# dtarb/TauDEM

Measured on AMD Instinct MI355X. Metric: Mcells/s (PitRemove->D8FlowDir->AreaD8 pipeline), higher is better.
Workload: dtype f32

## Files before the change

### taudem_amd/csrc/pitremove.hip

```cpp
#include "context.hpp"
#include "device_common.hpp"
#include "strips.hpp"
#include "tile_relax.hpp"

namespace {

constexpr int SEED_ROWS = 16;
constexpr int SEED_CF = 8;
template <int MODE>
__global__ __launch_bounds__(256) void pit_seed_kernel(const float* __restrict__ Z, const int16_t* __restrict__ mask,
                                                       float* __restrict__ W, int nx, int ny, int y_own0, int y_own1, float nodata, int step,
                                                       float* __restrict__ Zc, float* __restrict__ Wc, int nxc, int nyc, int nbx, int xmap) {
    const int bx = tdxk::xcd_block_x(nbx, xmap);
    if (bx < 0) return;
    const int x = bx * 64 + (threadIdx.x & 63);
    const int ybase = y_own0 + blockIdx.y * (4 * SEED_ROWS) + (threadIdx.x >> 6) * SEED_ROWS;
    const bool colok = x < nx;
    const int xc = colok ? x : nx - 1, xm = xc > 0 ? xc - 1 : xc, xp = xc < nx - 1 ? xc + 1 : xc;
    const int lane = int(threadIdx.x & 63);
    const bool edge_lane = lane == 0 || lane == 63;
    const int xe = lane == 0 ? xm : xp;
    float zm[SEED_ROWS + 2], zedge[SEED_ROWS + 2];
#pragma unroll
    for (int j = 0; j < SEED_ROWS + 2; j++) {
// ... 20 lines not shown
        const int l = tilek::lane_left(c, 0), r = tilek::lane_right(c, 0);
        nod[j] = in ? (unsigned(lane == 0 ? e : l) | (unsigned(c) << 1) | (unsigned(lane == 63 ? e : r) << 2)) : 7u;
    }
    float bmax[SEED_ROWS / SEED_CF];
    bool bany[SEED_ROWS / SEED_CF], bseed[SEED_ROWS / SEED_CF];
#pragma unroll
    for (int q = 0; q < SEED_ROWS / SEED_CF; q++) { bmax[q] = -FLT_MAX; bany[q] = false; bseed[q] = false; }
#pragma unroll
    for (int r = 0; r < SEED_ROWS; r++) {
        const int y = ybase + r;
        const float zc = zm[r + 1];
        const unsigned nn = nod[r], nc = nod[r + 1], ns = nod[r + 2];
        const bool c1 = (nc & 2u) != 0u;
        if (colok && y < y_own1) {
            const size_t idx = size_t(y) * size_t(nx) + size_t(x);
            float w;
            if (c1) w = TDX_FEL_NODATA;
            else if (mask && mask[idx] == 1) w = zc;
            else if (x == 0 || y == 0 || x == nx - 1 || y == ny - 1) w = zc;
            else {
                const bool con = (step == 2) ? (((nc & 5u) | (nn & 2u) | (ns & 2u)) != 0u) : ((nn | nc | ns) != 0u);
                w = con ? zc : FLT_MAX;
            }
            if (MODE == 0) W[idx] = w;
            if (MODE == 1 && !c1) {
                bany[r / SEED_CF] = true;
                bmax[r / SEED_CF] = fmaxf(bmax[r / SEED_CF], zc);
                if (w != FLT_MAX) bseed[r / SEED_CF] = true;
            }
            if (MODE == 2) {
                if (w == FLT_MAX) w = wc[r / SEED_CF];
                W[idx] = w;
            }
        }
    }
    if (MODE == 1) {
#pragma unroll
        for (int q = 0; q < SEED_ROWS / SEED_CF; q++) {
            float m = bmax[q];
            int fl = (bany[q] ? 1 : 0) | (bseed[q] ? 2 : 0);
#pragma unroll
            for (int off = 1; off < SEED_CF; off <<= 1) {
                m = fmaxf(m, __shfl_xor(m, off, 64));
                fl |= __shfl_xor(fl, off, 64);
            }
            const int yc = (ybase - y_own0) / SEED_CF + q, xcb = x / SEED_CF;
            if ((threadIdx.x & (SEED_CF - 1)) == 0 && xcb < nxc && yc < nyc) {
                const size_t c = size_t(yc) * size_t(nxc) + size_t(xcb);
                Zc[c] = (fl & 1) ? m : TDX_FEL_NODATA;
                Wc[c] = (fl & 1) ? ((fl & 2) ? m : FLT_MAX) : TDX_FEL_NODATA;
            }
        }
    }
}

constexpr int CF = 8;
static_assert(CF == SEED_CF, "pit_seed_kernel reduces to the first coarse level");
__global__ __launch_bounds__(256) void pit_coarsen_kernel(const float* __restrict__ Z, const float* __restrict__ W0, int nx, int ny, int nxc, int nyc,
                                                          float* __restrict__ Zc, float* __restrict__ Wc) {
// ... 89 lines not shown

template <int NBR>
struct PitOp {
    using T = float;
    static constexpr int kUniform = NBR;
    static constexpr int kWaves = 5;
    const float* Z;
    float* W;
    static __device__ __forceinline__ float inf() { return FLT_MAX; }
    using Raw = float;
    using CellRaw = float;
    __device__ __forceinline__ float load_raw(size_t idx) const { return W[idx]; }
    static __device__ __forceinline__ float decode(float v) { return v; }
    __device__ __forceinline__ void store(size_t idx, float v) const { W[idx] = v; }
    __device__ __forceinline__ float cell_raw(size_t idx) const { return Z[idx]; }
    static __device__ __forceinline__ void cell_decode(float z, float& cst, unsigned& mask) { cst = z; mask = (NBR == 4) ? 0x55u : 0xFFu; }
    static __device__ __forceinline__ float cell_floor(float z, float w) { return (w > z) ? z : w; }
    static __device__ __forceinline__ float apply(float z, float w, float m) { return tilek::med3_raw(z, w, m); }
    static __device__ __forceinline__ bool settled(float z, float w) { return !(w > z); }
    static __device__ __forceinline__ float act_never() { return -FLT_MAX; }
    static __device__ __forceinline__ float act_threshold(float z, float w) { return (w > z) ? w : act_never(); }
};

}

static int pit_finish_level(tdx_context* ctx, const Strip& ls, float* Zc, float* Wc, int nxc, int nyc, int64_t cells_all, tilek::Sched sc, int depth,
                            int64_t* rounds, int64_t* launches, int64_t* own_rounds = nullptr);

static inline Strip pit_level_strip(const Strip& st, int nxc, int nyc) {
    Strip ls;
    ls.nx = nxc; ls.comm = st.comm;
    if (st.multi()) { ls.ny_arr = nyc + 2; ls.y0 = 1; ls.y1 = nyc + 1; ls.up = st.up; ls.down = st.down; }
    else { ls.ny_arr = nyc; ls.y0 = 0; ls.y1 = nyc; }
    return ls;
}

template <int NBR>
static int pit_relax_level(tdx_context* ctx, const Strip& ls, const float* Z, float* W, tilek::Sched sc, int64_t* rounds, int64_t* launches, int64_t* outer,
                           bool all_tiles = true) {
    const tilek::TileGeom g = tilek::make_geom(ls.nx, ls.ny_arr, ls.y0, ls.y1);
    for (;;) {
        int rc = tile_relax_run(ctx, PitOp<NBR>{Z, W}, g, sc, rounds, launches, all_tiles);
        all_tiles = false;
        if (rc != TDX_OK) return rc;
        if (outer) (*outer)++;
        if (!ls.multi()) break;
        int64_t changed = 0;
        rc = strip_exchange<float>(ctx, ls, W, TDX_FEL_NODATA, sc.flags, g.tiles_x, &changed, true);
        if (rc != TDX_OK) return rc;
        if (changed == 0) break;
    }
    return TDX_OK;
}

static int pit_coarse_start(tdx_context* ctx, const Strip& st, const float* Z, float* W, int nx, int nyo, int64_t cells_all, tilek::Sched sc, int depth,
                            int64_t* rounds, int64_t* launches) {
    if (depth >= 3 || cells_all < (int64_t(1) << 18) || nyo < 1) return TDX_OK;
    hipStream_t s = ctx->stream;
    const int nxc = (nx + CF - 1) / CF, nyc = (nyo + CF - 1) / CF;
    const Strip ls = pit_level_strip(st, nxc, nyc);
    const size_t nc = size_t(nxc) * size_t(ls.ny_arr), off = size_t(ls.y0) * size_t(nxc);
    float* Zc = static_cast<float*>(ctx->scratch(TDX_S_D + 2 * depth, nc * 4));
    float* Wc = static_cast<float*>(ctx->scratch(TDX_S_E + 2 * depth, nc * 4));
    if (!Zc || !Wc) return TDX_ERR_NOMEM;
    const dim3 gc((nxc + 63) / 64, (nyc + 3) / 4);
// ... 24 lines not shown
    TDX_HIP_CHECK(ctx, hipSetDevice(ctx->device));
    hipStream_t s = ctx->stream;
    const tilek::TileGeom geom = tilek::make_geom(st.nx, st.ny_arr, st.y0, st.y1);
    const int ntiles = geom.tiles_x * geom.tiles_y;
    uint32_t* flags = static_cast<uint32_t*>(ctx->scratch(TDX_S_A, size_t(ntiles) * 4));
    uint32_t* list = static_cast<uint32_t*>(ctx->scratch(TDX_S_B, size_t(ntiles) * 4 * tilek::SCHED_LIST_WORDS));
    unsigned long long* counts = static_cast<unsigned long long*>(ctx->scratch(TDX_S_C, size_t(tilek::COUNT_RING) * 16));
    if (!flags || !list || !counts) return TDX_ERR_NOMEM;
    const tilek::Sched sched{flags, list, counts};

    ctx->begin_call(stats);
    strip_mark(ctx, st, "pitremove");
    int rc = strip_exchange<float>(ctx, st, d_dem, dem_nodata);
    if (rc != TDX_OK) return rc;
    int64_t rounds = 0, launches = 0, outer = 0;
    const int sbx = (st.nx + 63) / 64, sxmap = 0;
    const dim3 sgrid(unsigned(sbx), (st.y1 - st.y0 + 4 * SEED_ROWS - 1) / (4 * SEED_ROWS));
    const bool no_coarse = getenv("TDX_PIT_NO_COARSE") != nullptr;
    const int nyo = st.y1 - st.y0;
    int64_t cells_all = int64_t(st.nx) * int64_t(nyo);
    rc = strip_allreduce(ctx, st, &cells_all, 1, TDX_OP_SUM);
    if (rc != TDX_OK) return rc;
    const bool used_coarse = !fourway && !no_coarse && cells_all >= (int64_t(1) << 18);
    int64_t level1_rounds = 0;
    if (used_coarse) {
        const int nxc = (st.nx + CF - 1) / CF, nyc = (nyo + CF - 1) / CF;
        const Strip ls = pit_level_strip(st, nxc, nyc);
        const size_t nc = size_t(nxc) * size_t(ls.ny_arr), off = size_t(ls.y0) * size_t(nxc);
        float* Zc = static_cast<float*>(ctx->scratch(TDX_S_D, nc * 4));
        float* Wc = static_cast<float*>(ctx->scratch(TDX_S_E, nc * 4));
        if (!Zc || !Wc) return TDX_ERR_NOMEM;
        {
            TdxSpan sp(ctx, TDX_K_STENCIL);
            hipLaunchKernelGGL(pit_seed_kernel<1>, sgrid, dim3(256), 0, s, d_dem, d_mask, d_fel, st.nx, st.ny_arr, st.y0, st.y1, dem_nodata, 1, Zc + off, Wc + off, nxc, nyc, sbx, sxmap);
            if (stats) stats->launches[TDX_K_STENCIL]++;
        }
        {
            TdxSpan sp(ctx, TDX_K_RELAX);
            ctx->phase = "coarse levels";
            rc = pit_finish_level(ctx, ls, Zc, Wc, nxc, nyc, cells_all / (CF * CF), sched, 0, &rounds, &launches, &level1_rounds);
            if (rc != TDX_OK) return rc;
        }
        {
            TdxSpan sp(ctx, TDX_K_STENCIL);
            hipLaunchKernelGGL(pit_seed_kernel<2>, sgrid, dim3(256), 0, s, d_dem, d_mask, d_fel, st.nx, st.ny_arr, st.y0, st.y1, dem_nodata, 1, Zc + off, Wc + off, nxc, nyc, sbx, sxmap);
            if (stats) stats->launches[TDX_K_STENCIL]++;
        }
    } else {
        TdxSpan sp(ctx, TDX_K_STENCIL);
        hipLaunchKernelGGL(pit_seed_kernel<0>, sgrid, dim3(256), 0, s, d_dem, d_mask, d_fel, st.nx, st.ny_arr, st.y0, st.y1, dem_nodata, fourway ? 2 : 1,
                           static_cast<float*>(nullptr), static_cast<float*>(nullptr), 0, 0, sbx, sxmap);
        if (stats) stats->launches[TDX_K_STENCIL]++;
    }
    ctx->phase = "fine level";
    rc = strip_exchange<float>(ctx, st, d_fel, TDX_FEL_NODATA);
    if (rc != TDX_OK) return rc;
    {
        TdxSpan sp(ctx, TDX_K_RELAX);
        bool all_tiles = true;
        const int vc_env = getenv("TDX_PIT_VCYCLE_AFTER") ? std::max(0, atoi(getenv("TDX_PIT_VCYCLE_AFTER"))) : 8;
        if (used_coarse && vc_env > 0) {
            bool left = false;
            rc = tile_relax_run_bounded(ctx, PitOp<8>{d_dem, d_fel}, geom, sched, vc_env, &left, &rounds, &launches, true);
            if (rc != TDX_OK) return rc;
            all_tiles = false;
            const int vc_min = getenv("TDX_PIT_VCYCLE_MIN") ? atoi(getenv("TDX_PIT_VCYCLE_MIN")) : 16;
            if (st.multi() || (left && level1_rounds >= vc_min)) {
                const int nxc = (st.nx + CF - 1) / CF, nyc = (nyo + CF - 1) / CF;
                const Strip ls = pit_level_strip(st, nxc, nyc);
                const size_t off = size_t(ls.y0) * size_t(nxc);
                float* Zc = static_cast<float*>(ctx->scratch(TDX_S_D, size_t(nxc) * size_t(ls.ny_arr) * 4));
                float* Wc = static_cast<float*>(ctx->scratch(TDX_S_E, size_t(nxc) * size_t(ls.ny_arr) * 4));
                const tilek::TileGeom gc = tilek::make_geom(ls.nx, ls.ny_arr, ls.y0, ls.y1);
                const size_t ntc = size_t(gc.tiles_x) * size_t(gc.tiles_y);
                uint32_t* cflags = static_cast<uint32_t*>(ctx->scratch(TDX_S_L, ntc * 4 * (1 + tilek::SCHED_LIST_WORDS)));
                unsigned long long* ccounts = static_cast<unsigned long long*>(ctx->scratch(TDX_S_M, size_t(tilek::COUNT_RING) * 16));
                float* Ur = static_cast<float*>(ctx->scratch(TDX_S_N, size_t(nxc) * size_t(nyc) * 4));
                if (!Zc || !Wc || !cflags || !ccounts || !Ur) return TDX_ERR_NOMEM;
                ctx->phase = "coarse correction";
                TDX_HIP_CHECK(ctx, hipMemsetAsync(cflags, 0, ntc * 4, s));
                hipLaunchKernelGGL(pit_restrict_kernel, dim3((nxc + 63) / 64, (nyc + 3) / 4), dim3(256), 0, s, d_fel + size_t(st.y0) * size_t(st.nx), st.nx, nyo, nxc, nyc, Wc + off, Ur,
                                   ls.y0, ls.ny_arr, gc.tiles_x, cflags);
                {
                    int64_t changed = 0;
                    rc = strip_exchange<float>(ctx, ls, Wc, TDX_FEL_NODATA, cflags, gc.tiles_x, &changed);
                    if (rc != TDX_OK) return rc;
                }
                rc = pit_relax_level<8>(ctx, ls, Zc, Wc, tilek::Sched{cflags, cflags + ntc, ccounts}, &rounds, &launches, nullptr, false);
                if (rc != TDX_OK) return rc;
                hipLaunchKernelGGL(pit_prolong_min_kernel, dim3((st.nx + 63) / 64, (nyc + 3) / 4), dim3(256), 0, s, d_fel + size_t(st.y0) * size_t(st.nx), st.nx, nyo, Wc + off, Ur, nxc, nyc,
                                   st.y0, st.ny_arr, geom.tiles_x, flags);
                ctx->phase = "fine level";
                if (st.multi()) {
                    int64_t changed = 0;
                    rc = strip_exchange<float>(ctx, st, d_fel, TDX_FEL_NODATA, flags, geom.tiles_x, &changed);
                    if (rc != TDX_OK) return rc;
                }
            }
        }
        rc = fourway ? pit_relax_level<4>(ctx, st, d_dem, d_fel, sched, &rounds, &launches, &outer, all_tiles) : pit_relax_level<8>(ctx, st, d_dem, d_fel, sched, &rounds, &launches, &outer, all_tiles);
        if (rc != TDX_OK) return rc;
        if (stats) stats->launches[TDX_K_RELAX] += launches;
    }
    TDX_HIP_CHECK(ctx, hipGetLastError());
    if (stats) { stats->rounds = rounds; stats->cells_evaluated = outer; }
    ctx->end_call();
    return TDX_OK;
}

static int pitremove_check(tdx_context* ctx, const void* dem, const void* fel, int64_t nx, int64_t ny, int64_t halo, const char* who) {
    if (!ctx || !dem || !fel || nx <= 0 || ny <= 0) return tdx_fail(ctx, TDX_ERR_ARG, who);
    return too_big(nx, ny + halo) ? tdx_fail(ctx, TDX_ERR_ARG, "raster larger than 2^32 cells per device strip") : TDX_OK;
}

extern "C" int tdx_pitremove_dev(tdx_context* ctx, const float* d_dem, int64_t nx, int64_t ny, float dem_nodata,
                                 const int16_t* d_mask, int fourway, float* d_fel, tdx_stats* stats) {
    if (int rc = pitremove_check(ctx, d_dem, d_fel, nx, ny, 0, "tdx_pitremove_dev: bad argument")) return rc;
    return pitremove_impl(ctx, strip_single(int(nx), int(ny)), const_cast<float*>(d_dem), d_mask, fourway, dem_nodata, d_fel, stats);
}

extern "C" int tdx_pitremove_strip(tdx_context* ctx, const tdx_comm* comm, float* d_dem, int64_t nx, int64_t ny_local, float dem_nodata,
                                   const int16_t* d_mask, int fourway, float* d_fel, tdx_stats* stats) {
    if (int rc = pitremove_check(ctx, d_dem, d_fel, nx, ny_local, 2, "tdx_pitremove_strip: bad argument")) return rc;
// ... 14 lines not shown
```

### taudem_amd/csrc/tile_relax.hpp

```cpp
#pragma once
#include <atomic>
#include <algorithm>
#include <chrono>
#include <cstdlib>
#include <functional>
#include <type_traits>

#include "context.hpp"
#include "device_common.hpp"

namespace tilek {
using namespace tdxk;

constexpr int TS = 64;
constexpr int LH = TS + 2;
constexpr int LP = LH + 1;
constexpr int RPW = 16;
constexpr int NWAVE = TS / RPW;
constexpr int NTHR = NWAVE * 64;
constexpr int COUNT_RING = 1024;
constexpr int MAX_SWEEPS = 8;
constexpr int PULL_MAX = 64;
constexpr unsigned MACRO_DEAL_MAX = 4096;
constexpr unsigned MACRO_WGS_MIN = MACRO_DEAL_MAX / PULL_MAX;
// ... 67 lines not shown
    unsigned long long base;
    unsigned npend;
    int chain;
    uint32_t pulled[PULL_MAX];
    uint32_t pend[PULL_MAX * 9];
};

constexpr uint32_t FLAG_HALO = 1u, FLAG_FULL = 2u;
constexpr uint32_t TILE_IDX_MASK = 0x07ffffffu;
constexpr int TILE_BLK_SHIFT = 27;
__device__ __forceinline__ int entry_tile(uint32_t e) { return int(e & TILE_IDX_MASK); }
__device__ __forceinline__ int entry_blk_k(uint32_t e) { const unsigned c = (e >> TILE_BLK_SHIFT) & 3u; return c ? 1 << c : 0; }

__device__ __forceinline__ void activate_tiles_around(int x, int y, int nx, int ny, int tiles_x, uint32_t* __restrict__ tile_flags) {
#pragma unroll
    for (int dy = -1; dy <= 1; dy++)
#pragma unroll
        for (int dx = -1; dx <= 1; dx++) {
            const int xn = x + dx, yn = y + dy;
            if (xn >= 0 && xn < nx && yn >= 0 && yn < ny) tile_flags[(yn / TS) * tiles_x + xn / TS] = FLAG_FULL;
        }
}

constexpr int RES_CHANGED = 1 << 8;
constexpr int RES_CAPPED = 1 << 9;

template <class Op>
__device__ __forceinline__ int relax_tile(const Op& op, const TileGeom& g, int tile, bool full, typename Op::T* sV, TileLds& L, unsigned long long* __restrict__ dbg) {
    using T = typename Op::T;
    const int tid = threadIdx.x;
    const int lx = tid & 63;
    const int wv = tid >> 6;
    const int ry0 = wv * RPW;
        const int tx = tile % g.tiles_x, ty = tile / g.tiles_x;
        const int x0 = tx * TS, y0 = ty * TS;
        const unsigned long long tc0 = dbg ? __builtin_readcyclecounter() : 0ull;
        if (tid == 0) L.rim = 0;
        constexpr int NROWL = (LH + NWAVE - 1) / NWAVE;
        const int gx = x0 + lx;
        const bool col_ok = gx < g.nx;
        const int gxc = col_ok ? gx : g.nx - 1;
        const long long row_pitch = (long long)g.nx;
        typename Op::Raw stage[NROWL], stage_side;
        unsigned stage_ok = 0;
        bool side_ok = false;
        {
            int hy = y0 - 1 + wv;
#pragma unroll
            for (int i = 0; i < NROWL; i++) {
                const bool ok = col_ok && hy >= 0 && hy < g.ny && (wv + i * NWAVE < LH);
                const int hyc = hy < 0 ? 0 : (hy >= g.ny ? g.ny - 1 : hy);
                stage[i] = op.load_raw(size_t((long long)hyc * row_pitch + gxc));
// ... 322 lines not shown
    y |= __builtin_amdgcn_update_dpp(0, y, 0x118, 0xf, 0xf, true);
    return unsigned(__builtin_amdgcn_readlane(y, 15) | __builtin_amdgcn_readlane(y, 31) | __builtin_amdgcn_readlane(y, 47) | __builtin_amdgcn_readlane(y, 63));
}

template <class Op, class = void>
struct has_act_threshold : std::false_type {};
template <class Op>
struct has_act_threshold<Op, std::void_t<decltype(Op::act_never())>> : std::true_type {};
template <class Op, class = void>
struct has_act_threshold_raw : std::false_type {};
template <class Op>
struct has_act_threshold_raw<Op, std::void_t<decltype(Op::act_threshold_raw(typename Op::Raw()))>> : std::true_type {};
template <class T>
__device__ __forceinline__ T max_t(T a, T b) { return a > b ? a : b; }
template <class Op, class = void>
struct has_raw_can_move : std::false_type {};
template <class Op>
struct has_raw_can_move<Op, std::void_t<decltype(Op::raw_can_move(typename Op::Raw()))>> : std::true_type {};
struct NoCellRaw {};
template <class Op, class = void>
struct cell_raw_of { using type = NoCellRaw; static constexpr bool value = false; };
template <class Op>
struct cell_raw_of<Op, std::void_t<typename Op::CellRaw>> { using type = typename Op::CellRaw; static constexpr bool value = true; };

template <class Op>
__device__ __forceinline__ int relax_tile_reg(const Op& op, const TileGeom& g, int tile, typename Op::T* sV, TileLds& L, unsigned long long* __restrict__ dbg) {
    using T = typename Op::T;
    const int tid = threadIdx.x;
    const int lx = tid & 63;
    const int wv = tid >> 6;
    const int ry0 = wv * RPW;
    const int tx = tile % g.tiles_x, ty = tile / g.tiles_x;
    const int x0 = tx * TS, y0 = ty * TS;
    T* sSide = sV;
    T* sRow = sV + 2 * LH;
    const unsigned long long tc0 = dbg ? __builtin_readcyclecounter() : 0ull;
    if (tid == 0) L.rim = 0;
    if (lx == 0) L.rows[wv] = 0u;
    const int gx = x0 + lx;
    const bool col_ok = gx < g.nx;
    const int gxc = col_ok ? gx : g.nx - 1;
    const long long row_pitch = (long long)g.nx;
    typename Op::Raw raw[RPW], raw_edge, raw_side;
    constexpr bool kCellRaw = cell_raw_of<Op>::value;
    typename cell_raw_of<Op>::type craw[RPW], craw_edge = {};
    {
        int gy = y0 + ry0;
#pragma unroll
        for (int r = 0; r < RPW; r++) {
            const int gyc = gy >= g.ny ? g.ny - 1 : gy;
            const size_t idx = size_t((long long)gyc * row_pitch + gxc);
            raw[r] = op.load_raw(idx);
            if constexpr (kCellRaw) craw[r] = op.cell_raw(idx);
            gy++;
        }
    }
    const int ey = (wv == 0) ? y0 - 1 : y0 + TS;
    const bool edge_ok = col_ok && ey >= 0 && ey < g.ny;
    bool side_ok;
    {
        const int eyc = ey < 0 ? 0 : (ey >= g.ny ? g.ny - 1 : ey);
        raw_edge = op.load_raw(size_t((long long)eyc * row_pitch + gxc));
        if constexpr (has_act_threshold<Op>::value && !has_act_threshold_raw<Op>::value) craw_edge = op.cell_raw(size_t((long long)eyc * row_pitch + gxc));
        const int row = (tid >> 1) < LH ? (tid >> 1) : LH - 1, right = tid & 1;
        const int sx = right ? x0 + TS : x0 - 1, sy = y0 - 1 + row;
        side_ok = tid < 2 * LH && sx >= 0 && sx < g.nx && sy >= 0 && sy < g.ny;
        const int sxc = sx < 0 ? 0 : (sx >= g.nx ? g.nx - 1 : sx), syc = sy < 0 ? 0 : (sy >= g.ny ? g.ny - 1 : sy);
        raw_side = op.load_raw(size_t((long long)syc * row_pitch + sxc));
    }
    T v[RPW], cst[RPW];
    unsigned mk[RPW / 4] = {};
    unsigned live = 0;
#pragma unroll
    for (int r = 0; r < RPW; r++) {
        const int gy = y0 + ry0 + r;
        v[r] = (col_ok && gy < g.ny) ? Op::decode(raw[r]) : Op::inf();
        T c = Op::inf();
        unsigned m = 0;
        bool movable = col_ok && gy >= g.y_own0 && gy < g.y_own1;
        if constexpr (has_raw_can_move<Op>::value) movable = movable && Op::raw_can_move(raw[r]);
        if (movable) {
            if constexpr (kCellRaw) Op::cell_decode(craw[r], c, m);
            else Op::cell_decode(c, m);
        }
        if (m && !Op::settled(c, v[r])) live |= 1u << r;
        cst[r] = Op::cell_floor(c, v[r]);
        mk[r >> 2] |= (m & 0xFFu) << (8 * (r & 3));
    }
    const T edge_row = edge_ok ? Op::decode(raw_edge) : Op::inf();
    if (tid < 2 * LH) sSide[(tid & 1) * LH + (tid >> 1)] = side_ok ? Op::decode(raw_side) : Op::inf();
    T* sEdgeT = sRow + 2 * NWAVE * 2 * TS;
// ... 63 lines not shown
        sRow[(((cur ^ 1) * NWAVE + wv) * 2 + 1) * TS + lx] = v[RPW - 1];
        if (lx == 0) {
            L.any[cur][wv] = chg_rows != 0u;
            L.top[cur][wv] = chg_rows & 1u;
            L.bot[cur][wv] = (chg_rows >> (RPW - 1)) & 1u;
        }
        __syncthreads();
        unsigned any = 0;
#pragma unroll
        for (int w = 0; w < NWAVE; w++) any |= L.any[cur][w];
        if (any) any_change = true;
        if (!any || iter + 1 >= g.max_sweeps) {
            capped = any != 0;
            if (dbg && tid == 0) { atomicAdd(dbg, (unsigned long long)(iter + 1)); atomicAdd(dbg + 1, 1ull); }
            break;
        }
        unsigned nd = (chg_rows | (chg_rows << 1) | (chg_rows >> 1)) & ((1u << RPW) - 1u);
        const unsigned above = wv > 0 ? unsigned(L.bot[cur][wv > 0 ? wv - 1 : 0]) : 0u, below = wv < NWAVE - 1 ? unsigned(L.top[cur][wv < NWAVE - 1 ? wv + 1 : 0]) : 0u;
        if (above) nd |= 1u;
        if (below) nd |= 1u << (RPW - 1);
        rows = __builtin_amdgcn_readfirstlane(nd) & rows_live;
    }
    const unsigned long long tc2 = dbg ? __builtin_readcyclecounter() : 0ull;
    if (any_change) {
        if constexpr (has_act_threshold_raw<Op>::value) {
            int rim = 0;
            const int wvu = __builtin_amdgcn_readfirstlane(wv);
            const bool all = g.act_filter == 0;
            if (wvu == 0 && __ballot((moved & 1u) != 0u && (all || v[0] < sEdgeT[lx])) != 0ull) rim |= 1;
            if (wvu == NWAVE - 1 && __ballot(((moved >> (RPW - 1)) & 1u) != 0u && (all || v[RPW - 1] < sEdgeT[TS + lx])) != 0ull) rim |= 2;
            T* sCol = sRow;
            if (lx == 0 || lx == TS - 1) {
                T* col = sCol + (lx ? TS : 0) + ry0;
#pragma unroll
                for (int r = 0; r < RPW; r++) col[r] = ((moved >> r) & 1u) ? v[r] : Op::inf();
            }
            __syncthreads();
            size_t idx = size_t(y0 + ry0) * size_t(g.nx) + size_t(gx);
#pragma unroll
            for (int r = 0; r < RPW; r++) {
                if ((moved >> r) & 1u) op.store(idx, v[r]);
                idx += size_t(g.nx);
            }
            if (wvu < 2) {
                const T val = sCol[wvu * TS + lx];
                const T* st = sSideT + wvu * LH;
// ... 209 lines not shown
    }
    for (unsigned base = bid; base < nact; base += nblocks * 64u) {
        __syncthreads();
        if (threadIdx.x == 0) L.next = 0u;
        __syncthreads();
        if (threadIdx.x < 64u) {
            const unsigned i = base + nblocks * threadIdx.x;
            const uint32_t e = i < nact ? list[i] : 0u;
            if (i < nact && entry_blk_k(e)) L.pulled[atomicAdd(&L.next, 1u)] = e;
        }
        __syncthreads();
        const unsigned nb = L.next;
        if (dbg && threadIdx.x == 0 && nb) atomicMax(dbg + 15, (unsigned long long)nb);
        serve(nb);
    }
}

template <class Op, bool REG>
__global__ __launch_bounds__(NTHR, relax_waves<Op>::value) void relax_kernel(Op op, TileGeom g, const uint32_t* __restrict__ list, unsigned long long* __restrict__ count,
                                                    uint32_t* __restrict__ flags_cur, uint32_t* __restrict__ flags_next,
                                                    uint32_t* __restrict__ list_next, unsigned pull_max, unsigned long long* __restrict__ dbg, unsigned grid_tiles) {
    using T = typename Op::T;
    static_assert(sizeof(T) == 4, "tile engine works on 4-byte values");
    constexpr int kLdsWords = REG ? (REG_LDS_WORDS > macro_lds_words<Op>::value ? REG_LDS_WORDS : macro_lds_words<Op>::value) : LH * LP;
    __shared__ T sV[kLdsWords];
    __shared__ TileLds L;
    if constexpr (REG && has_macro<Op>::value) {
        if (grid_tiles != 0u && blockIdx.x >= grid_tiles) {
            macro_role(op, g, list, count, flags_next, list_next, reinterpret_cast<int*>(sV), L, blockIdx.x - grid_tiles, gridDim.x - grid_tiles, dbg);
            return;
        }
    }
    const unsigned nblocks = grid_tiles != 0u ? grid_tiles : gridDim.x;
    round_driver(list, count, flags_cur, flags_next, list_next, pull_max, g, L, [&](int tile, bool full) {
        if constexpr (REG && has_plain<Op>::value) {
            if (!__builtin_amdgcn_readfirstlane(int(op.tile_masked(tile)))) return relax_tile_reg(op.plain(), g, tile, sV, L, dbg);
        }
        return REG ? relax_tile_reg(op, g, tile, sV, L, dbg) : relax_tile(op, g, tile, full, sV, L, dbg);
    }, blockIdx.x, nblocks);
}

struct RoundArgs { const uint32_t* list; unsigned long long* count; uint32_t* flags_cur; uint32_t* flags_next; uint32_t* list_next; };
template <class Op>
__global__ __launch_bounds__(NTHR, relax_waves<Op>::value) void relax_pair_kernel(Op opA, Op opB, TileGeom g, RoundArgs a, RoundArgs b, unsigned gridA,
                                                                                  unsigned pull_max) {
    using T = typename Op::T;
    static_assert(sizeof(T) == 4, "tile engine works on 4-byte values");
    __shared__ T sV[REG_LDS_WORDS];
    __shared__ TileLds L;
    const bool second = blockIdx.x >= gridA;
    const Op op = second ? opB : opA;
    const RoundArgs ra = second ? b : a;
    round_driver(ra.list, ra.count, ra.flags_cur, ra.flags_next, ra.list_next, pull_max, g, L,
                 [&](int tile, bool) {
                     if constexpr (has_plain<Op>::value) {
                         if (!__builtin_amdgcn_readfirstlane(int(op.tile_masked(tile)))) return relax_tile_reg(op.plain(), g, tile, sV, L, nullptr);
                     }
                     return relax_tile_reg(op, g, tile, sV, L, nullptr);
                 },
                 second ? blockIdx.x - gridA : blockIdx.x, second ? gridDim.x - gridA : gridA);
}
// ... 204 lines not shown
    TDX_HIP_CHECK(ctx, hipMemsetAsync(sc.counts, 0, 8 * sizeof(unsigned long long), s));
    TDX_HIP_CHECK(ctx, hipMemsetAsync(ring, 0, size_t(cap) * 4, s));
    hipLaunchKernelGGL(async_fill_kernel, dim3(cgrid), dim3(256), 0, s, sc.flags, ntiles, c, count);
    hipLaunchKernelGGL(async_start_kernel, dim3(1), dim3(1), 0, s, c, count);
    const unsigned grid = unsigned(std::min(ntiles, 4 * ctx->num_cus));
    hipLaunchKernelGGL((relax_async_kernel<Op>), dim3(grid), dim3(NTHR), 0, s, op, g, c, dbg);
    TDX_HIP_CHECK(ctx, hipMemcpyAsync(host_mail, sc.counts, 4 * sizeof(unsigned long long), hipMemcpyDeviceToHost, s));
    TDX_HIP_CHECK(ctx, hipStreamSynchronize(s));
    const unsigned err = unsigned(host_mail[3] & 0xffffffffull);
    *gave_up = err != 0;
    if (err) {
        fprintf(stderr, "taudem_amd: asynchronous tile worklist gave up (code %u, head %llu tail %llu pending %d); continuing with the round schedule\n", err,
                (unsigned long long)host_mail[0], (unsigned long long)host_mail[1], int(host_mail[2] & 0xffffffffull));
        hipLaunchKernelGGL(fill_u32_kernel, dim3(cgrid), dim3(256), 0, s, sc.flags, FLAG_FULL, size_t(ntiles));
    }
    return TDX_OK;
}

struct RoundSchedule {
    using Launch = std::function<void(const tilek::TileGeom& rg, unsigned grid, hipStream_t st, const uint32_t* list, unsigned long long* count, uint32_t* flags_cur,
                                      uint32_t* flags_next, uint32_t* list_next, unsigned pull_max)>;
    tdx_context* ctx; hipStream_t s; tilek::TileGeom g; tilek::Sched sc; uint64_t* h;
    Launch launch;
    int ntiles; unsigned cgrid, grid_full, grid_small;
    bool print_counts = false;
    int ring_len;
    bool lds_variant;
    unsigned pull_max;
    int r = 0, parity = 0, batch = 4;
    int r_enq = 0, parity_enq = 0, n_enq = 0, n_col = 0, fl_batch[2] = {0, 0};
    bool polled[2] = {false, false};
    uint64_t fl_tag[2] = {0, 0};
    int ev_base = 0;
    int batch_max = 64;
    bool done = false;
    int64_t rounds = 0, launches = 0;
    bool short_tail = getenv("TDX_RELAX_LONG_TAIL") == nullptr;
    unsigned long long last_count = 0;
    RoundSchedule(tdx_context* c, hipStream_t st, tilek::TileGeom geom, tilek::Sched sched, uint64_t* host_mail, Launch l = nullptr)
        : ctx(c), s(st), g(geom), sc(sched), h(host_mail), launch(std::move(l)) {
        ntiles = g.tiles_x * g.tiles_y;
        cgrid = tdx_blocks_for(size_t(ntiles), 256);
        grid_full = unsigned(std::min(ntiles, 8 * ctx->num_cus));
        static const int gs_env = getenv("TDX_RELAX_GRID_SMALL") ? std::max(1, atoi(getenv("TDX_RELAX_GRID_SMALL"))) : 0;
        grid_small = unsigned(std::min(ntiles, gs_env ? gs_env : ctx->num_cus));
        const char* e = getenv("TDX_RELAX_RING");
// ... 33 lines not shown
        if (batch < 1) batch = 1;
        if (r_enq + batch + 1 > ring_len) {
            hipLaunchKernelGGL(ring_wrap_kernel, dim3(1), dim3(256), 0, s, sc.counts, r_enq);
            r_enq = 0;
        }
        const int slot = n_enq & 1;
        uint64_t* hs = h + slot * TDX_MAIL_RUN_SLOT;
        const int r = r_enq, parity = parity_enq;
        const bool timed = ctx->kernel_timing && s == ctx->stream;
        const unsigned grid = (rounds > 0 && last_count <= 256ull) ? grid_small : grid_full;
        static const bool count_copy = getenv("TDX_RELAX_COUNT_COPY") != nullptr;
        if (!count_copy) {
            uint32_t seq = ++ctx->run_seq;
            if (seq == 0xffffffffu) seq = ++ctx->run_seq;
            fl_tag[slot] = uint64_t(seq) << 32;
            for (int b = 0; b < batch; b++) hs[b] = ~0ull;
            g.cnt_host = reinterpret_cast<unsigned long long*>(hs);
            g.cnt_dev = sc.counts + r;
            g.cnt_tag = fl_tag[slot];
        } else { g.cnt_host = nullptr; g.cnt_dev = nullptr; g.cnt_tag = 0ull; }
        for (int b = 0; b < batch; b++) {
            const int p = (parity + b) & 1;
            const int sp = timed ? ctx->span_begin(TDX_K_TILEK) : -1;
            launch(g, grid, s, list_of(p), sc.counts + r + b, flags_of(p), flags_of(p ^ 1), list_of(p ^ 1), pull_max);
            ctx->span_end(sp);
            if (timed && ctx->cur_stats) ctx->cur_stats->launches[TDX_K_TILEK]++;
        }
        launches += batch;
        fl_batch[slot] = batch;
        polled[slot] = !count_copy;
        if (count_copy) {
            TDX_HIP_CHECK(ctx, hipMemcpyAsync(hs, sc.counts + r, size_t(batch) * sizeof(unsigned long long), hipMemcpyDeviceToHost, s));
            hipEvent_t& ev = ctx->ev_batch[ev_base + slot];
            if (!ev) TDX_HIP_CHECK(ctx, hipEventCreateWithFlags(&ev, hipEventDisableTiming));
            TDX_HIP_CHECK(ctx, hipEventRecord(ev, s));
        }
        r_enq += batch;
        parity_enq = (parity_enq + batch) & 1;
        n_enq++;
        if (batch < batch_max) batch = std::min(2 * batch, batch_max);
        if (short_tail && rounds > 0 && last_count <= 8ull) batch = std::min(batch, 4);
        static const int tail_batch = getenv("TDX_RELAX_TAIL_BATCH") ? std::max(2, atoi(getenv("TDX_RELAX_TAIL_BATCH"))) : 0;
        if (tail_batch && rounds > 0 && last_count <= 256ull) batch = std::min(batch, tail_batch);
        return TDX_OK;
    }
    int wait_oldest() {
        const int slot = n_col & 1;
// ... 48 lines not shown
            rc = wait_oldest();
            if (rc != TDX_OK) return rc;
            collect();
        }
        return TDX_OK;
    }
};

template <class Op>
struct RoundRunner : RoundSchedule {
    Op op; unsigned long long* dbg;
    RoundRunner(tdx_context* c, hipStream_t st, Op o, tilek::TileGeom geom, tilek::Sched sched, uint64_t* host_mail, unsigned long long* d)
        : RoundSchedule(c, st, geom, sched, host_mail), op(o), dbg(d) {
        launch = [this](const tilek::TileGeom& rg, unsigned grid, hipStream_t ls, const uint32_t* list, unsigned long long* count, uint32_t* fcur, uint32_t* fnext,
                        uint32_t* lnext, unsigned pm) {
            using namespace tilek;
            if (lds_variant)
                hipLaunchKernelGGL((relax_kernel<Op, false>), dim3(grid), dim3(NTHR), 0, ls, op, rg, list, count, fcur, fnext, lnext, pm, dbg, 0u);
            else {
                static const int macro_wgs = getenv("TDX_MACRO_WGS") ? std::max(1, atoi(getenv("TDX_MACRO_WGS"))) : 4;
                const unsigned gm = (has_macro<Op>::value && rg.blk_k != nullptr) ? std::max(unsigned(macro_wgs * ctx->num_cus), MACRO_WGS_MIN) : 0u;
                hipLaunchKernelGGL((relax_kernel<Op, true>), dim3(grid + gm), dim3(NTHR), 0, ls, op, rg, list, count, fcur, fnext, lnext, pm, dbg, gm ? grid : 0u);
            }
        };
    }
};

template <class Op>
static int enqueue_fused(RoundRunner<Op>& A, RoundRunner<Op>& B) {
    using namespace tilek;
    tdx_context* ctx = A.ctx;
    hipStream_t s = A.s;
    static const long long round_cap = getenv("TDX_RELAX_MAX_ROUNDS") ? atoll(getenv("TDX_RELAX_MAX_ROUNDS")) : 0;
    if (std::max(A.rounds, B.rounds) > (round_cap > 0 ? round_cap : 64ll * A.ntiles + 65536ll))
        return tdx_fail(ctx, TDX_ERR_HIP, "tile schedule: no fixed point after " + std::to_string(std::max(A.rounds, B.rounds)) + " rounds (" + std::to_string(A.ntiles) + " tiles)");
    int batch = std::min(A.batch, A.ring_len - 2);
    if (A.r_enq + batch + 1 > A.ring_len) {
        hipLaunchKernelGGL(ring_wrap_kernel, dim3(1), dim3(256), 0, s, A.sc.counts, A.r_enq);
        hipLaunchKernelGGL(ring_wrap_kernel, dim3(1), dim3(256), 0, s, B.sc.counts, B.r_enq);
        A.r_enq = B.r_enq = 0;
    }
    const int slot = A.n_enq & 1, r = A.r_enq, parity = A.parity_enq;
    auto grid_of = [](const RoundRunner<Op>& R) { return R.done ? 0u : ((R.rounds > 0 && R.last_count <= 256ull) ? R.grid_small : R.grid_full); };
    const unsigned gA = grid_of(A), gB = grid_of(B);
    for (int b = 0; b < batch; b++) {
        const int p = (parity + b) & 1;
// ... 61 lines not shown
    A.prestarted = B.prestarted = flags0 != nullptr;
    A.batch_max = B.batch_max = RoundSchedule::pipelined_batch_max();
    int rc = A.start();
    if (rc != TDX_OK) return rc;
    rc = B.start();
    if (rc != TDX_OK) return rc;
    rc = A.enqueue();
    if (rc != TDX_OK) return rc;
    rc = B.enqueue();
    if (rc != TDX_OK) return rc;
    while (!A.done || !B.done) {
        if (!A.done) { rc = A.enqueue(); if (rc != TDX_OK) return rc; }
        if (!B.done) { rc = B.enqueue(); if (rc != TDX_OK) return rc; }
        if (!A.done) { rc = A.wait_oldest(); if (rc != TDX_OK) return rc; A.collect(); }
        if (!B.done) { rc = B.wait_oldest(); if (rc != TDX_OK) return rc; B.collect(); }
    }
    TDX_HIP_CHECK(ctx, hipEventRecord(ctx->ev_fork, ctx->stream2));
    TDX_HIP_CHECK(ctx, hipStreamWaitEvent(ctx->stream, ctx->ev_fork, 0));
    if (rounds_out) *rounds_out += A.rounds + B.rounds;
    if (launches_out) *launches_out += A.launches + B.launches;
    return TDX_OK;
}

template <class Op>
static int tile_relax_run_bounded(tdx_context* ctx, Op op, tilek::TileGeom g, tilek::Sched sc, int max_rounds, bool* active_left, int64_t* rounds_out,
                                  int64_t* launches_out, bool all_tiles = false) {
    RoundRunner<Op> run(ctx, ctx->stream, op, g, sc, ctx->h_mail + TDX_MAIL_RUN_A, nullptr);
    run.all_tiles = all_tiles;
    run.batch = run.batch_max = std::max(2, std::min(max_rounds, 64));
    static const int debug_level = getenv("TDX_DEBUG_ROUNDS") ? atoi(getenv("TDX_DEBUG_ROUNDS")) : 0;
    run.print_counts = debug_level > 0;
    if (debug_level == 2) fprintf(stderr, "\nrounds(%d tiles, at most %d):", run.ntiles, max_rounds);
    *active_left = false;
    int rc = run.start();
    if (rc != TDX_OK) return rc;
    while (!run.done) {
        rc = run.enqueue();
        if (rc != TDX_OK) return rc;
        rc = run.wait_oldest();
        if (rc != TDX_OK) return rc;
        run.collect();
        if (!run.done && run.rounds >= max_rounds) { *active_left = true; break; }
    }
    if (*active_left && run.parity)
        hipLaunchKernelGGL(tilek::flags_fold_kernel, dim3(tdx_blocks_for(size_t(run.ntiles), 256)), dim3(256), 0, ctx->stream, run.flags_of(0), run.flags_of(1), run.ntiles);
    if (rounds_out) *rounds_out += run.rounds;
    if (launches_out) *launches_out += run.launches;
    return TDX_OK;
}

template <class Op>
static int tile_relax_run(tdx_context* ctx, Op op, tilek::TileGeom g, tilek::Sched sc, int64_t* rounds_out, int64_t* launches_out, bool all_tiles = false) {
    using namespace tilek;
    hipStream_t s = ctx->stream;
    const int ntiles = g.tiles_x * g.tiles_y;
    static const int debug_level = getenv("TDX_DEBUG_ROUNDS") ? atoi(getenv("TDX_DEBUG_ROUNDS")) : 0;
    static const bool debug = debug_level == 1;
    static const bool force_rounds = getenv("TDX_RELAX_ASYNC") == nullptr;
    unsigned long long* dbg = nullptr;
    if (debug) {
        dbg = reinterpret_cast<unsigned long long*>(ctx->d_mail) + TDX_MAIL_DBG_RELAX;
        TDX_HIP_CHECK(ctx, hipMemsetAsync(dbg, 0, 128, s));
    }
    int64_t rounds = 0, launches = 0;
    bool need_rounds = force_rounds;
    if (!force_rounds) {
        bool gave_up = false;
        int rc = tile_relax_async_finish(ctx, s, op, g, sc, TDX_S_Q, ctx->h_mail, dbg, &gave_up);
        if (rc != TDX_OK) return rc;
        launches += 1;
        rounds += 1;
        need_rounds = gave_up;
    }
    if (need_rounds) {
        RoundRunner<Op> run(ctx, s, op, g, sc, ctx->h_mail + TDX_MAIL_RUN_A, dbg);
        run.all_tiles = all_tiles && force_rounds;
        run.print_counts = debug_level > 0;
        if (debug_level == 2) fprintf(stderr, "\nrounds(%d tiles):", ntiles);
        int rc = run.drive();
        if (rc != TDX_OK) return rc;
        rounds += run.rounds;
        launches += run.launches;
    }
    if (debug) {
        TDX_HIP_CHECK(ctx, hipMemcpyAsync(ctx->h_mail, dbg, 128, hipMemcpyDeviceToHost, s));
        TDX_HIP_CHECK(ctx, hipStreamSynchronize(s));
        fprintf(stderr, "tile_relax_run(%d tiles, %s): %lld rounds, %llu tile activations, %llu sweeps; queue pops %llu pushes %llu activations %llu\n", ntiles,
                need_rounds ? "rounds" : "worklist", (long long)rounds, (unsigned long long)ctx->h_mail[1], (unsigned long long)ctx->h_mail[0],
                (unsigned long long)ctx->h_mail[2], (unsigned long long)ctx->h_mail[3], (unsigned long long)ctx->h_mail[4]);
        const double na = double(ctx->h_mail[1] ? ctx->h_mail[1] : 1);
        fprintf(stderr, "    cycles per activation (s_memtime): load %.0f, sweeps %.0f, write-back %.0f\n", double(ctx->h_mail[6]) / na, double(ctx->h_mail[7]) / na,
                double(ctx->h_mail[8]) / na);
        fprintf(stderr, "    load split: issue tile loads %.0f, issue cell loads %.0f, wait+LDS stores %.0f, barrier %.0f\n", double(ctx->h_mail[9]) / na,
                double(ctx->h_mail[10]) / na, double(ctx->h_mail[11]) / na, double(ctx->h_mail[12]) / na);
        if (ctx->h_mail[14]) fprintf(stderr, "    macro blocks: %llu updates, %.0f cycles each (offers %.0f, stores + gain test %.0f, activations %.0f), at most %llu per workgroup and look\n",
                                    (unsigned long long)ctx->h_mail[14], double(ctx->h_mail[13]) / double(ctx->h_mail[14]), double(ctx->h_mail[9]) / double(ctx->h_mail[14]),
                                    double(ctx->h_mail[10]) / double(ctx->h_mail[14]), double(ctx->h_mail[11]) / double(ctx->h_mail[14]), (unsigned long long)ctx->h_mail[15]);
    }
    if (rounds_out) *rounds_out += rounds;
// ... 4 lines not shown
```

Before: 13860.

## Fuse coarse-fill seed pass into first fine relaxation launch

The coarse seeding kernel now writes the fine seed values and the coarse aggregates in a single pass (MODE 3). The second seeding pass, which filled unset cells from the coarse solution, is dropped. That fill now happens inside the first fine-level tile relaxation launch through a PitStartOp, which reads coarse values per band and writes back filled cells even when relaxation leaves them unchanged. The aim is to save one full-grid read/write pass and a kernel launch. The cost is extra coarse loads, LDS space and register pressure in the first relaxation kernel, plus separate halo prolongation for multi-strip runs.

New measurement: 14010, median of 6. +1.1%, better.

```diff
diff --git a/taudem_amd/csrc/pitremove.hip b/taudem_amd/csrc/pitremove.hip
--- a/taudem_amd/csrc/pitremove.hip
+++ b/taudem_amd/csrc/pitremove.hip
@@ -1,3 +1,5 @@
+#include <cstring>
+
 #include "context.hpp"
 #include "device_common.hpp"
 #include "strips.hpp"
@@ -66,8 +68,8 @@
                 const bool con = (step == 2) ? (((nc & 5u) | (nn & 2u) | (ns & 2u)) != 0u) : ((nn | nc | ns) != 0u);
                 w = con ? zc : FLT_MAX;
             }
-            if (MODE == 0) W[idx] = w;
-            if (MODE == 1 && !c1) {
+            if (MODE == 0 || MODE == 3) W[idx] = w;
+            if ((MODE == 1 || MODE == 3) && !c1) {
                 bany[r / SEED_CF] = true;
                 bmax[r / SEED_CF] = fmaxf(bmax[r / SEED_CF], zc);
                 if (w != FLT_MAX) bseed[r / SEED_CF] = true;
@@ -78,7 +80,7 @@
             }
         }
     }
-    if (MODE == 1) {
+    if (MODE == 1 || MODE == 3) {
 #pragma unroll
         for (int q = 0; q < SEED_ROWS / SEED_CF; q++) {
             float m = bmax[q];
@@ -214,6 +216,56 @@
     static __device__ __forceinline__ float act_threshold(float z, float w) { return (w > z) ? w : act_never(); }
 };
 
+struct PitStartOp : PitOp<8> {
+    static constexpr int kWaves = 4;
+    const float* Wc;
+    int nxc, ny_arr_c, cy0, nyc;
+    int y_own0, y_own1;
+    struct Fill { float v[4]; bool aligned; };
+    __device__ __forceinline__ int coarse_row(int y) const { return y >= y_own1 ? cy0 + nyc : cy0 + ((y - y_own0) >> 3); }
+    __device__ __forceinline__ float coarse_at(int x, int cr) const {
+        const int crc = cr < 0 ? 0 : (cr >= ny_arr_c ? ny_arr_c - 1 : cr);
+        return Wc[size_t(crc) * size_t(nxc) + size_t(x / CF)];
+    }
+    __device__ __forceinline__ Fill fill_load(int x, int y) const {
+        Fill f;
+        const int c0 = coarse_row(y);
+#pragma unroll
+        for (int q = 0; q < 4; q++) f.v[q] = coarse_at(x, c0 + q);
+        f.aligned = y >= y_own0 && ((y - y_own0) & (CF - 1)) == 0 && y + tilek::RPW <= y_own1;
+        return f;
+    }
+    __device__ __forceinline__ unsigned fill_band(const Fill& f, float (&w)[tilek::RPW], int y) const {
+        static_assert(CF == 8 && tilek::RPW == 2 * CF, "two block rows per band");
+        unsigned ch = 0;
+        if (f.aligned) {
+#pragma unroll
+            for (int r = 0; r < tilek::RPW; r++) {
+                const float nw = w[r] == FLT_MAX ? f.v[r / CF] : w[r];
+                ch = tilek::shift_in_ne(ch, nw, w[r]);
+                w[r] = nw;
+            }
+        } else {
+            const int c0 = coarse_row(y);
+#pragma unroll
+            for (int r = 0; r < tilek::RPW; r++) {
+                const int q = coarse_row(y + r) - c0;
+                const bool m = w[r] == FLT_MAX;
+                float nw = w[r];
+                nw = (m && q == 0) ? f.v[0] : nw;
+                nw = (m && q == 1) ? f.v[1] : nw;
+                nw = (m && q == 2) ? f.v[2] : nw;
+                nw = (m && q == 3) ? f.v[3] : nw;
+                ch = tilek::shift_in_ne(ch, nw, w[r]);
+                w[r] = nw;
+            }
+        }
+        return __builtin_bitreverse32(ch) >> (32 - tilek::RPW);
+    }
+    __device__ __forceinline__ float fill_cell(int x, int y) const { return coarse_at(x, coarse_row(y)); }
+    static __device__ __forceinline__ float fill(float w, float wc) { return w == FLT_MAX ? wc : w; }
+};
+
 }
 
 static int pit_finish_level(tdx_context* ctx, const Strip& ls, float* Zc, float* Wc, int nxc, int nyc, int64_t cells_all, tilek::Sched sc, int depth,
@@ -229,10 +281,11 @@
 
 template <int NBR>
 static int pit_relax_level(tdx_context* ctx, const Strip& ls, const float* Z, float* W, tilek::Sched sc, int64_t* rounds, int64_t* launches, int64_t* outer,
-                           bool all_tiles = true) {
+                           bool all_tiles = true, const PitStartOp* start = nullptr) {
     const tilek::TileGeom g = tilek::make_geom(ls.nx, ls.ny_arr, ls.y0, ls.y1);
     for (;;) {
-        int rc = tile_relax_run(ctx, PitOp<NBR>{Z, W}, g, sc, rounds, launches, all_tiles);
+        int rc = tile_relax_run(ctx, PitOp<NBR>{Z, W}, g, sc, rounds, launches, all_tiles, all_tiles ? start : nullptr);
+        start = nullptr;
         all_tiles = false;
         if (rc != TDX_OK) return rc;
         if (outer) (*outer)++;
@@ -303,6 +356,9 @@
     rc = strip_allreduce(ctx, st, &cells_all, 1, TDX_OP_SUM);
     if (rc != TDX_OK) return rc;
     const bool used_coarse = !fourway && !no_coarse && cells_all >= (int64_t(1) << 18);
+    const char* seed_env = getenv("TDX_PIT_SEED");
+    const bool one_seed_pass = used_coarse && !(seed_env && strcmp(seed_env, "two") == 0) && !getenv("TDX_RELAX_LDS") && !getenv("TDX_RELAX_ASYNC");
+    PitStartOp start_op{{d_dem, d_fel}, nullptr, 0, 0, 0, 0, st.y0, st.y1};
     int64_t level1_rounds = 0;
     if (used_coarse) {
         const int nxc = (st.nx + CF - 1) / CF, nyc = (nyo + CF - 1) / CF;
@@ -313,8 +369,12 @@
         if (!Zc || !Wc) return TDX_ERR_NOMEM;
         {
             TdxSpan sp(ctx, TDX_K_STENCIL);
-            hipLaunchKernelGGL(pit_seed_kernel<1>, sgrid, dim3(256), 0, s, d_dem, d_mask, d_fel, st.nx, st.ny_arr, st.y0, st.y1, dem_nodata, 1, Zc + off, Wc + off, nxc, nyc, sbx, sxmap);
+            if (one_seed_pass)
+                hipLaunchKernelGGL(pit_seed_kernel<3>, sgrid, dim3(256), 0, s, d_dem, d_mask, d_fel, st.nx, st.ny_arr, st.y0, st.y1, dem_nodata, 1, Zc + off, Wc + off, nxc, nyc, sbx, sxmap);
+            else
+                hipLaunchKernelGGL(pit_seed_kernel<1>, sgrid, dim3(256), 0, s, d_dem, d_mask, d_fel, st.nx, st.ny_arr, st.y0, st.y1, dem_nodata, 1, Zc + off, Wc + off, nxc, nyc, sbx, sxmap);
             if (stats) stats->launches[TDX_K_STENCIL]++;
+            start_op.Wc = Wc; start_op.nxc = nxc; start_op.ny_arr_c = ls.ny_arr; start_op.cy0 = ls.y0; start_op.nyc = nyc;
         }
         {
             TdxSpan sp(ctx, TDX_K_RELAX);
@@ -322,7 +382,7 @@
             rc = pit_finish_level(ctx, ls, Zc, Wc, nxc, nyc, cells_all / (CF * CF), sched, 0, &rounds, &launches, &level1_rounds);
             if (rc != TDX_OK) return rc;
         }
-        {
+        if (!one_seed_pass) {
             TdxSpan sp(ctx, TDX_K_STENCIL);
             hipLaunchKernelGGL(pit_seed_kernel<2>, sgrid, dim3(256), 0, s, d_dem, d_mask, d_fel, st.nx, st.ny_arr, st.y0, st.y1, dem_nodata, 1, Zc + off, Wc + off, nxc, nyc, sbx, sxmap);
             if (stats) stats->launches[TDX_K_STENCIL]++;
@@ -336,14 +396,21 @@
     ctx->phase = "fine level";
     rc = strip_exchange<float>(ctx, st, d_fel, TDX_FEL_NODATA);
     if (rc != TDX_OK) return rc;
+    if (one_seed_pass && st.multi()) {
+        const dim3 gh((st.nx + 63) / 64, 1);
+        hipLaunchKernelGGL(pit_prolong_kernel, gh, dim3(256), 0, s, d_fel, st.nx, 1, start_op.Wc + size_t(start_op.cy0 - 1) * size_t(start_op.nxc), start_op.nxc);
+        hipLaunchKernelGGL(pit_prolong_kernel, gh, dim3(256), 0, s, d_fel + size_t(st.y1) * size_t(st.nx), st.nx, 1,
+                           start_op.Wc + size_t(start_op.cy0 + start_op.nyc) * size_t(start_op.nxc), start_op.nxc);
+    }
     {
         TdxSpan sp(ctx, TDX_K_RELAX);
-        bool all_tiles = true;
+        bool all_tiles = true, first_run_done = false;
         const int vc_env = getenv("TDX_PIT_VCYCLE_AFTER") ? std::max(0, atoi(getenv("TDX_PIT_VCYCLE_AFTER"))) : 8;
         if (used_coarse && vc_env > 0) {
             bool left = false;
-            rc = tile_relax_run_bounded(ctx, PitOp<8>{d_dem, d_fel}, geom, sched, vc_env, &left, &rounds, &launches, true);
+            rc = tile_relax_run_bounded(ctx, PitOp<8>{d_dem, d_fel}, geom, sched, vc_env, &left, &rounds, &launches, true, one_seed_pass ? &start_op : nullptr);
             if (rc != TDX_OK) return rc;
+            first_run_done = true;
             all_tiles = false;
             const int vc_min = getenv("TDX_PIT_VCYCLE_MIN") ? atoi(getenv("TDX_PIT_VCYCLE_MIN")) : 16;
             if (st.multi() || (left && level1_rounds >= vc_min)) {
@@ -379,7 +446,8 @@
                 }
             }
         }
-        rc = fourway ? pit_relax_level<4>(ctx, st, d_dem, d_fel, sched, &rounds, &launches, &outer, all_tiles) : pit_relax_level<8>(ctx, st, d_dem, d_fel, sched, &rounds, &launches, &outer, all_tiles);
+        rc = fourway ? pit_relax_level<4>(ctx, st, d_dem, d_fel, sched, &rounds, &launches, &outer, all_tiles)
+                     : pit_relax_level<8>(ctx, st, d_dem, d_fel, sched, &rounds, &launches, &outer, all_tiles, (one_seed_pass && !first_run_done) ? &start_op : nullptr);
         if (rc != TDX_OK) return rc;
         if (stats) stats->launches[TDX_K_RELAX] += launches;
     }
diff --git a/taudem_amd/csrc/tile_relax.hpp b/taudem_amd/csrc/tile_relax.hpp
--- a/taudem_amd/csrc/tile_relax.hpp
+++ b/taudem_amd/csrc/tile_relax.hpp
@@ -113,12 +113,19 @@
         }
 }
 
+struct NoFill {};
+template <class Op, class = void>
+struct start_fill_of { using type = NoFill; static constexpr bool value = false; };
+template <class Op>
+struct start_fill_of<Op, std::void_t<typename Op::Fill>> { using type = typename Op::Fill; static constexpr bool value = true; };
+
 constexpr int RES_CHANGED = 1 << 8;
 constexpr int RES_CAPPED = 1 << 9;
 
 template <class Op>
 __device__ __forceinline__ int relax_tile(const Op& op, const TileGeom& g, int tile, bool full, typename Op::T* sV, TileLds& L, unsigned long long* __restrict__ dbg) {
     using T = typename Op::T;
+    static_assert(!start_fill_of<Op>::value, "a start operator (Op::Fill) has the register form only");
     const int tid = threadIdx.x;
     const int lx = tid & 63;
     const int wv = tid >> 6;
@@ -487,7 +494,6 @@
 struct cell_raw_of { using type = NoCellRaw; static constexpr bool value = false; };
 template <class Op>
 struct cell_raw_of<Op, std::void_t<typename Op::CellRaw>> { using type = typename Op::CellRaw; static constexpr bool value = true; };
-
 template <class Op>
 __device__ __forceinline__ int relax_tile_reg(const Op& op, const TileGeom& g, int tile, typename Op::T* sV, TileLds& L, unsigned long long* __restrict__ dbg) {
     using T = typename Op::T;
@@ -520,6 +526,11 @@
             gy++;
         }
     }
+    constexpr bool kFill = start_fill_of<Op>::value;
+    typename start_fill_of<Op>::type fill_rows = {};
+    typename Op::Raw fill_edge = {}, fill_side = {};
+    int fy0 = 0;
+    if constexpr (kFill) { fy0 = __builtin_amdgcn_readfirstlane(y0 + ry0); fill_rows = op.fill_load(gxc, fy0); }
     const int ey = (wv == 0) ? y0 - 1 : y0 + TS;
     const bool edge_ok = col_ok && ey >= 0 && ey < g.ny;
     bool side_ok;
@@ -527,11 +538,22 @@
         const int eyc = ey < 0 ? 0 : (ey >= g.ny ? g.ny - 1 : ey);
         raw_edge = op.load_raw(size_t((long long)eyc * row_pitch + gxc));
         if constexpr (has_act_threshold<Op>::value && !has_act_threshold_raw<Op>::value) craw_edge = op.cell_raw(size_t((long long)eyc * row_pitch + gxc));
+        if constexpr (kFill) fill_edge = op.fill_cell(gxc, __builtin_amdgcn_readfirstlane(eyc));
         const int row = (tid >> 1) < LH ? (tid >> 1) : LH - 1, right = tid & 1;
         const int sx = right ? x0 + TS : x0 - 1, sy = y0 - 1 + row;
         side_ok = tid < 2 * LH && sx >= 0 && sx < g.nx && sy >= 0 && sy < g.ny;
         const int sxc = sx < 0 ? 0 : (sx >= g.nx ? g.nx - 1 : sx), syc = sy < 0 ? 0 : (sy >= g.ny ? g.ny - 1 : sy);
         raw_side = op.load_raw(size_t((long long)syc * row_pitch + sxc));
+        if constexpr (kFill) fill_side = op.fill_cell(sxc, syc);
+    }
+    if constexpr (kFill) {
+        static_assert(!has_act_threshold_raw<Op>::value && !has_raw_can_move<Op>::value, "the fill is written for the per-row write-back");
+        const int lo = g.y_own0 - fy0 < 0 ? 0 : (g.y_own0 - fy0 > RPW ? RPW : g.y_own0 - fy0), hi = g.y_own1 - fy0 < 0 ? 0 : (g.y_own1 - fy0 > RPW ? RPW : g.y_own1 - fy0);
+        const unsigned own_rows = hi > lo ? (((1u << hi) - 1u) & ~((1u << lo) - 1u)) : 0u;
+        const unsigned filled = col_ok ? (op.fill_band(fill_rows, raw, fy0) & own_rows) : 0u;
+        raw_edge = Op::fill(raw_edge, fill_edge);
+        raw_side = Op::fill(raw_side, fill_side);
+        reinterpret_cast<unsigned*>(sV + REG_LDS_WORDS)[tid] = filled;
     }
     T v[RPW], cst[RPW];
     unsigned mk[RPW / 4] = {};
@@ -641,6 +663,17 @@
         rows = __builtin_amdgcn_readfirstlane(nd) & rows_live;
     }
     const unsigned long long tc2 = dbg ? __builtin_readcyclecounter() : 0ull;
+    if constexpr (kFill) {
+        const unsigned only = reinterpret_cast<const unsigned*>(sV + REG_LDS_WORDS)[tid] & ~moved;
+        if (__ballot(only != 0u) != 0ull) {
+            size_t idx = size_t(y0 + ry0) * size_t(g.nx) + size_t(gx);
+#pragma unroll
+            for (int r = 0; r < RPW; r++) {
+                if ((only >> r) & 1u) op.store(idx, v[r]);
+                idx += size_t(g.nx);
+            }
+        }
+    }
     if (any_change) {
         if constexpr (has_act_threshold_raw<Op>::value) {
             int rim = 0;
@@ -896,7 +929,7 @@
                                                     uint32_t* __restrict__ list_next, unsigned pull_max, unsigned long long* __restrict__ dbg, unsigned grid_tiles) {
     using T = typename Op::T;
     static_assert(sizeof(T) == 4, "tile engine works on 4-byte values");
-    constexpr int kLdsWords = REG ? (REG_LDS_WORDS > macro_lds_words<Op>::value ? REG_LDS_WORDS : macro_lds_words<Op>::value) : LH * LP;
+    constexpr int kLdsWords = REG ? (REG_LDS_WORDS > macro_lds_words<Op>::value ? REG_LDS_WORDS : macro_lds_words<Op>::value) + (start_fill_of<Op>::value ? NTHR : 0) : LH * LP;
     __shared__ T sV[kLdsWords];
     __shared__ TileLds L;
     if constexpr (REG && has_macro<Op>::value) {
@@ -910,7 +943,8 @@
         if constexpr (REG && has_plain<Op>::value) {
             if (!__builtin_amdgcn_readfirstlane(int(op.tile_masked(tile)))) return relax_tile_reg(op.plain(), g, tile, sV, L, dbg);
         }
-        return REG ? relax_tile_reg(op, g, tile, sV, L, dbg) : relax_tile(op, g, tile, full, sV, L, dbg);
+        if constexpr (REG) return relax_tile_reg(op, g, tile, sV, L, dbg);
+        else return relax_tile(op, g, tile, full, sV, L, dbg);
     }, blockIdx.x, nblocks);
 }
 
@@ -1161,6 +1195,7 @@
                                       uint32_t* flags_next, uint32_t* list_next, unsigned pull_max)>;
     tdx_context* ctx; hipStream_t s; tilek::TileGeom g; tilek::Sched sc; uint64_t* h;
     Launch launch;
+    Launch first_launch;
     int ntiles; unsigned cgrid, grid_full, grid_small;
     bool print_counts = false;
     int ring_len;
@@ -1240,7 +1275,7 @@
         for (int b = 0; b < batch; b++) {
             const int p = (parity + b) & 1;
             const int sp = timed ? ctx->span_begin(TDX_K_TILEK) : -1;
-            launch(g, grid, s, list_of(p), sc.counts + r + b, flags_of(p), flags_of(p ^ 1), list_of(p ^ 1), pull_max);
+            ((first_launch && launches == 0 && b == 0) ? first_launch : launch)(g, grid, s, list_of(p), sc.counts + r + b, flags_of(p), flags_of(p ^ 1), list_of(p ^ 1), pull_max);
             ctx->span_end(sp);
             if (timed && ctx->cur_stats) ctx->cur_stats->launches[TDX_K_TILEK]++;
         }
@@ -1335,6 +1370,15 @@
                 const unsigned gm = (has_macro<Op>::value && rg.blk_k != nullptr) ? std::max(unsigned(macro_wgs * ctx->num_cus), MACRO_WGS_MIN) : 0u;
                 hipLaunchKernelGGL((relax_kernel<Op, true>), dim3(grid + gm), dim3(NTHR), 0, ls, op, rg, list, count, fcur, fnext, lnext, pm, dbg, gm ? grid : 0u);
             }
+        };
+    }
+    template <class StartOp>
+    void start_with(StartOp sop) {
+        static_assert(tilek::start_fill_of<StartOp>::value, "a start operator");
+        first_launch = [this, sop](const tilek::TileGeom& rg, unsigned grid, hipStream_t ls, const uint32_t* list, unsigned long long* count, uint32_t* fcur, uint32_t* fnext,
+                                   uint32_t* lnext, unsigned pm) {
+            using namespace tilek;
+            hipLaunchKernelGGL((relax_kernel<StartOp, true>), dim3(grid), dim3(NTHR), 0, ls, sop, rg, list, count, fcur, fnext, lnext, pm, dbg, 0u);
         };
     }
 };
@@ -1442,11 +1486,12 @@
     return TDX_OK;
 }
 
-template <class Op>
+template <class Op, class StartOp = Op>
 static int tile_relax_run_bounded(tdx_context* ctx, Op op, tilek::TileGeom g, tilek::Sched sc, int max_rounds, bool* active_left, int64_t* rounds_out,
-                                  int64_t* launches_out, bool all_tiles = false) {
+                                  int64_t* launches_out, bool all_tiles = false, const StartOp* start = nullptr) {
     RoundRunner<Op> run(ctx, ctx->stream, op, g, sc, ctx->h_mail + TDX_MAIL_RUN_A, nullptr);
     run.all_tiles = all_tiles;
+    if constexpr (tilek::start_fill_of<StartOp>::value) { if (start) run.start_with(*start); }
     run.batch = run.batch_max = std::max(2, std::min(max_rounds, 64));
     static const int debug_level = getenv("TDX_DEBUG_ROUNDS") ? atoi(getenv("TDX_DEBUG_ROUNDS")) : 0;
     run.print_counts = debug_level > 0;
@@ -1469,8 +1514,9 @@
     return TDX_OK;
 }
 
-template <class Op>
-static int tile_relax_run(tdx_context* ctx, Op op, tilek::TileGeom g, tilek::Sched sc, int64_t* rounds_out, int64_t* launches_out, bool all_tiles = false) {
+template <class Op, class StartOp = Op>
+static int tile_relax_run(tdx_context* ctx, Op op, tilek::TileGeom g, tilek::Sched sc, int64_t* rounds_out, int64_t* launches_out, bool all_tiles = false,
+                          const StartOp* start = nullptr) {
     using namespace tilek;
     hipStream_t s = ctx->stream;
     const int ntiles = g.tiles_x * g.tiles_y;
@@ -1484,7 +1530,8 @@
     }
     int64_t rounds = 0, launches = 0;
     bool need_rounds = force_rounds;
-    if (!force_rounds) {
+    if (start != nullptr) need_rounds = true;
+    else if (!force_rounds) {
         bool gave_up = false;
         int rc = tile_relax_async_finish(ctx, s, op, g, sc, TDX_S_Q, ctx->h_mail, dbg, &gave_up);
         if (rc != TDX_OK) return rc;
@@ -1494,7 +1541,8 @@
     }
     if (need_rounds) {
         RoundRunner<Op> run(ctx, s, op, g, sc, ctx->h_mail + TDX_MAIL_RUN_A, dbg);
-        run.all_tiles = all_tiles && force_rounds;
+        run.all_tiles = all_tiles && (force_rounds || start != nullptr);
+        if constexpr (tilek::start_fill_of<StartOp>::value) { if (start) run.start_with(*start); }
         run.print_counts = debug_level > 0;
         if (debug_level == 2) fprintf(stderr, "\nrounds(%d tiles):", ntiles);
         int rc = run.drive();
```
